# Russoul/cuda-mat

Hardware: AMD Instinct MI355X
Metric: BiCGSTAB iters/sec + SpMV effective HBM GB/s, 10M-row CSR at 1/2/4/8 GPUs (higher is better)
Workload: dtype f64

## Files before the change

### cuda_mat_amd/csrc/config.cpp

```cpp
#include "config.h"

#include <stdio.h>
#include <stdlib.h>
#include <string.h>

#include <unistd.h>

#include <mutex>
#include <set>
#include <string>

extern char **environ;

#include "common.h"

namespace cm {

namespace {

enum Kind { K_FLAG, K_INT, K_LLONG, K_ENUM, K_FAIL };

struct Option {
    const char *name;
    Kind kind;
// ... 14 lines not shown
    OPT_ENUM("SPMV_MODE", spmv_mode, "csr=0,pb=1,sell=2,pat=3", "force the CSR forms / the blocked two-phase form / SELL-C-sigma / the row-pattern dictionary"),
    OPT_FLAG("SPMV_SELL", spmv_sell, "0: keep SELL-C-sigma out of the candidates"),
    OPT_ENUM("SPMV_FORM", spmv_form, "lanes=1,tiles=2", "inside the CSR forms: lanes per row / nnz-balanced tiles"),
    OPT_INT("SPMV_LANES", spmv_lanes, 2, 64, "lanes per row, a power of two (and no stream tiles)"),
    OPT_FLAG("SPMV_COMPRESS", spmv_compress, "0: stream kernel on the plain 32-bit indices"),
    OPT_FLAG("SPMV_ALIGN", spmv_align, "0: compressed stream kernel without line-aligned copies of its value / offset streams"),
    OPT_ENUM("SPMV_TUNE", spmv_tune_full, "full=1", "time every SpMV candidate even when the column span already decides"),
    OPT_FLAG("VALUE_DICT", value_dict, "0: keep fp64 values even when the matrix has <= 256 distinct ones"),
    OPT_INT("PB_MIN_WAVES", pb_min_waves, 256, 1 << 20, "blocked form: fewest phase-2 waves"),
    OPT_INT("PB_DEPTH", pb_depth, 4, 16, "blocked form: segment loads in flight per phase-2 wave (4, 8 or 16)"),
    OPT_FLAG("POOL", pool, "0: device memory straight from hipMalloc / hipFree instead of the library's recycling pool (read once per process)"),
    OPT_FLAG("SKIP_ORIG_COPY", skip_orig_copy, "0: cudamat_solve with ILU(0) builds the blocked copy in the original index space even when its loop will run in the level-major spaces"),
    OPT_FLAG("EARLY_ANALYSIS", early_analysis, "0: cudamat_solve analyses the ILU(0) levels after the upload of the values instead of beside it"),
    OPT_INT("PB_FILL_OCC", pb_fill_occ, 0, 64, "resident waves per CU of the two-pass fill's first pass (0: 8; probing)"),
    OPT_FLAG("PB_FILL2", pb_fill2, "0: fill the blocked copy with the single-pass scatter kernel (rounds 1-4) instead of the two-pass partition"),
    OPT_INT("PB_PLACE", pb_place, 0, 2, "blocked copy of a large matrix: 1 (default): a resident solver's product stream is placed in a memory class of its own, values and indices in another (timed probe of the device's memory classes, 10-35 ms per copy: spmv_pb.hip); 2: the drop-in calls place theirs as well; 0: arrays wherever the allocator puts them"),
    OPT_INT("PB_PLACE_MAX_MS", pb_place_max_ms, 0, 60000, "PB_PLACE: what the search for an arrangement may take before the arrays are allocated as ever (ms; the slabs it allocates included -- 0.3 ms per 16 GB on most boxes, 2 s on some)"),
    OPT_FLAG("PB_PROBE_FAIL", pb_probe_fail, "1 (tests): treat the run-time LDS-order probe as failed, i.e. select the architected-order phase 2"),
    OPT_FLAG("PB_STRICT", pb_strict, "1: phase 2 adds a row's products of one wave instruction rank by rank (architected order, +10 %)"),
    {"FUSED", K_LLONG, nullptr, &Config::fused, 0, 1LL << 40, nullptr,
     "0: never fold the vector updates into the SpMVs (three launches per iteration); N: do it for every supported plan up to N rows"},
    OPT_FLAG("RESIDENT", resident, "0: never run the whole loop of a very small system in one launch"),
    OPT_INT("RESIDENT_SPIN_LIMIT", resident_spin_limit, 0, 1 << 30, "polls a grid-barrier wait of the single-launch loop may take"),
    OPT_FLAG("GUARD", guard, "1: every solve on the context runs as if CUDAMAT_FLAG_GUARD were set: restart from the true residual when rho has lost its last bit, converged = 1 only for a verified iterate (reference loops, one GPU)"),
    {"GUARD_RHO_ULPS", K_LLONG, nullptr, &Config::guard_rho_ulps, 1, 1LL << 52, nullptr,
     "guarded solves restart when |rho| <= N * 2^-52 * sum |rw_i r_i| (default 4; 2^52 fires at every iteration >= 1: tests)"},
    OPT_INT("PIPE_RR", pipe_rr, 0, 1 << 20, "residual replacement period of the pipelined loop (0: never)"),
    OPT_FLAG("TRSV_SYNCFREE", trsv_syncfree, "0: one launch per level; 1: dependency-driven launches also for narrow levels"),
    OPT_FLAG("TRSV_LDS", trsv_lds, "0: no single-workgroup LDS-resident triangular solve for small systems"),
    OPT_FLAG("TRSV_HYBRID", trsv_hybrid, "0 | 1: never / always split big factors into far (blocked SpMV) and near (dependency-driven) parts"),
// ... 151 lines not shown
```

### cuda_mat_amd/csrc/config.h

```cpp
#pragma once

namespace cm {

struct Config {
    int verbose = 0;
    int roctx = 0;
    int spmv_mode = -1;
    int spmv_sell = 1;
    int spmv_form = 0;
    int spmv_lanes = 0;
    int spmv_compress = 1;
    int spmv_align = 1;
    int spmv_tune_full = 0;
    int value_dict = 1;
    int pb_min_waves = 0;
    int pb_depth = 0;
    int pool = 1;
    int skip_orig_copy = 1;
    int early_analysis = 1;
    int pb_fill_occ = 0;
    int pb_fill2 = 1;
    int pb_place = 1;
    int pb_place_max_ms = 300;
    int pb_probe_fail = 0;
    int pb_strict = 0;
    long long fused = -1;
    int resident = 1;
    int resident_spin_limit = -1;
    int guard = 0;
    long long guard_rho_ulps = 4;
    int pipe_rr = -1;
    int trsv_syncfree = -1;
    int trsv_lds = 1;
    int trsv_hybrid = -1;
    int trsv_groups = 0;
    int trsv_lanes = 0;
// ... 26 lines not shown
```

### cuda_mat_amd/csrc/spmv_pb.h

```cpp
#pragma once
#include "kernels.h"
#include "valdict.h"

namespace cm {

constexpr int kPbMaxChunks = 16;

struct PbCols {
    int64_t per = 0;
    int chunks = 1;
    int rank = 0;
};

struct PbPlan {
    int n = 0;
    int64_t n_cols = 0;
    int64_t nnz = 0;
    int CB = 0, NCB = 0;
    int64_t per = 0;
    int chunks = 1;
    int64_t chunk_len = 0;
    int bpc = 0;
    int RB = 0, NRB = 0;
    int NW = 0;
    int SR = 0;
    int LPS = 64;
    int depth = 4;
    int NSUB = 0;
    double *pv = nullptr;
    unsigned char *pvi = nullptr;
    const double *dict = nullptr;
    int ndict = 0;
    unsigned short *pc = nullptr;
    unsigned short *pr = nullptr;
    double *P = nullptr;
    int *cstart = nullptr;
    int *col0 = nullptr;
    int *sstart = nullptr;
    int *slen = nullptr;
    int *order = nullptr;
    int part_off[kPbMaxChunks + 2] = {0};
    int placed = -1;
    int place_slabs = 0;
    double place_seconds = 0.0;
    float place_check_ms = 0.f, place_fast_ms = 0.f, place_slow_ms = 0.f;
    char place_classes[192] = {0};
    bool pc_zeroed = false;
    double build_seconds = 0.0;
};

struct PbCut {
    int per, chunks, chunk_len, bpc, CB;
};
struct PbBuild {
    PbPlan p;
    int *bins = nullptr;
    PbCut cut{};
    size_t cap = 0;
    double t0 = 0.0;
    bool verbose = false;
    bool two_pass = false;
    int place = 0;
    bool report_classes = false;
    double place_max_seconds = 0.3;
    int fill_occ = 0;
    int GB = 1, NG = 1;
    unsigned long long *smeta = nullptr;
    int *gstart = nullptr;
};
int pb_build_begin(hipStream_t st, const Config &cfg, int n, int64_t n_cols, int64_t nnz, const int *rp, const int *ci,
                   const PbCols *cols, PbBuild *b);
int pb_build_alloc(hipStream_t st, const Config &cfg, int n, int64_t n_cols, int64_t nnz, const PbCols *cols, PbBuild *b);
int pb_build_count(hipStream_t st, const Config &cfg, const int *rp, const int *ci, PbBuild *b);
// ... 17 lines not shown
```

### cuda_mat_amd/csrc/spmv_pb.hip

```cpp
#include <algorithm>
#include <map>
#include <mutex>
#include <string>
#include <vector>

#include "device.h"
#include "spmv_pb.h"

namespace cm {

typedef unsigned short u16;
constexpr int kPbBuildWaves = 4;
constexpr int kP1Threads = 1024;
constexpr int kP1Unroll = 8;
constexpr int kTileMax = 13312;
constexpr int kPbAlign = 64;

void pb_free(PbPlan *p)
{
    void *ptrs[] = {p->pv, p->pvi, p->pc, p->pr, p->P, p->cstart, p->col0, p->sstart, p->slen, p->order};
    for (void *q : ptrs)
        if (q) CM_DROP(hipFree(q));
    *p = PbPlan();
}

bool pb_candidate(hipStream_t st, int n, int64_t n_cols, int64_t nnz, const int *rp, const int *ci)
{
    (void)st; (void)rp; (void)ci;
    if (n < 65536 || nnz < (1 << 20) || n_cols * 8 < (1 << 20)) return false;
    if ((double)nnz / n < 4.0) return false;
    if ((int64_t)n > (int64_t)kMaxParts * kTileMax) return false;
    return true;
}

__device__ __forceinline__ int col_to_cb(const PbCut &c, int col)
// ... 17 lines not shown
__device__ __forceinline__ int wave_match_rank(unsigned long long *tab, int key, bool active, int lane, int nkeys, int *count_of_key_lane)
{
    if (lane < nkeys) tab[lane] = 0ULL;
    __builtin_amdgcn_fence(__ATOMIC_RELEASE, "wavefront");
    __builtin_amdgcn_wave_barrier();
    if (active) atomicOr(&tab[key], 1ULL << lane);
    __builtin_amdgcn_fence(__ATOMIC_RELEASE, "wavefront");
    __builtin_amdgcn_wave_barrier();
    const unsigned long long mine = active ? tab[key] : 0ULL;
    *count_of_key_lane = lane < nkeys ? __popcll(tab[lane]) : 0;
    __builtin_amdgcn_fence(__ATOMIC_RELEASE, "wavefront");
    __builtin_amdgcn_wave_barrier();
    return __popcll(mine & ((1ULL << lane) - 1ULL));
}

template <bool FILL>
__global__ __launch_bounds__(64 * kPbBuildWaves) void k_pb_rows(int n, const int *rp, const int *ci,
                                                               const double *val, PbCut cut, const int *col0, int NCB,
                                                               int SR, int NSUB, int *bins, double *pv, u16 *pc, u16 *pr,
                                                               const unsigned char *vidx, unsigned char *pvi, int sub0, int sub1)
{
    extern __shared__ int lds_i[];
    const int wave = threadIdx.x >> 6, lane = threadIdx.x & 63;
    const int sub = sub0 + blockIdx.x * kPbBuildWaves + wave;
    if (sub >= sub1) return;
    int *cur = lds_i + (size_t)wave * NCB;
    for (int c = lane; c < NCB; c += 64) cur[c] = FILL ? bins[(size_t)c * NSUB + sub] : 0;
    __builtin_amdgcn_fence(__ATOMIC_RELEASE, "wavefront");
    __builtin_amdgcn_wave_barrier();
    const long long row0 = (long long)sub * SR;
    const int row1 = (int)(row0 + SR < n ? row0 + SR : n);
    for (int row = (int)row0; row < row1; row++) {
        const int rs = rp[row], re = rp[row + 1];
        for (int k0 = rs; k0 < re; k0 += 64) {
            const int k = k0 + lane;
// ... 6 lines not shown
#pragma unroll
            for (int o = 1; o < 64; o <<= 1) {
                const int t = __shfl_up(hs, o, 64);
                if (lane >= o) hs = t > hs ? t : hs;
            }
            const int next = __shfl_down(cb, 1, 64);
            const bool tail = lane == 63 || next != cb;
            if (active) {
                const int base = cur[cb];
                const int rank = lane - hs;
                if (FILL) {
                    const int dest = base + rank;
                    if (pvi) pvi[dest] = vidx[k];
                    else pv[dest] = val[k];
                    pc[dest] = (u16)(col - col0[cb]);
                    pr[dest] = (u16)(row - (int)row0);
                }
                if (tail) cur[cb] = base + rank + 1;
            }
            __builtin_amdgcn_fence(__ATOMIC_RELEASE, "wavefront");
            __builtin_amdgcn_wave_barrier();
        }
    }
    if (!FILL)
        for (int c = lane; c < NCB; c += 64) bins[(size_t)c * NSUB + sub] = cur[c];
}

constexpr int kPbGroups = 32;
static_assert(kPbGroups <= 64, "one lane per group");
constexpr int kPbRpMax = 2047;
constexpr int kPbBucketMax = 2048;
// ... 98 lines not shown
        run += added;
        if (active) {
            if (sval8) sval8[dest] = vi;
            else sval[dest] = v;
            smeta[dest] = pb_pack(cb, col - (one_piece ? cb * cut.CB : col0[cb]), r);
        }
        const unsigned long long am = __ballot(active);
        rbase = __builtin_amdgcn_readlane(r, 63 - __builtin_clzll(am));
    }
}

constexpr int kPbScatterWaves = 4;
__global__ __launch_bounds__(64 * kPbScatterWaves) void k_pb_scatter(int NCB, int NSUB, const int *slen, const int *bins, int GB, int NG,
                                                                    const int *gstart, const double *sval, const unsigned char *sval8,
                                                                    const unsigned long long *smeta, double *pv, unsigned char *pvi,
                                                                    u16 *pc, u16 *pr, int sub0, int sub1)
{
    __shared__ unsigned raw_all[kPbScatterWaves][kPbBucketMax];
    __shared__ unsigned char cbl_all[kPbScatterWaves][kPbBucketMax];
    __shared__ u16 inv_all[kPbScatterWaves][kPbBucketMax];
    __shared__ unsigned long long tab_all[kPbScatterWaves][64];
    const int wave = threadIdx.x >> 6, lane = threadIdx.x & 63;
    const long long bucket = (long long)blockIdx.x * kPbScatterWaves + wave;
    const int sub = sub0 + (int)(bucket / NG), g = (int)(bucket % NG);
    if (sub >= sub1) return;
    u16 *inv = inv_all[wave];
    unsigned *raw = raw_all[wave];
    unsigned char *cbs = cbl_all[wave];
    const int start = gstart[(size_t)sub * (NG + 1) + g], len = gstart[(size_t)sub * (NG + 1) + g + 1] - start;
    if (len <= 0) return;
    const int cbid = g * GB + lane;
    const bool owner = lane < GB && cbid < NCB;
    const int cnt = owner ? slen[(size_t)sub * NCB + cbid] : 0;
    int inc = cnt;
#pragma unroll
    for (int o = 1; o < 64; o <<= 1) {
        const int t = __shfl_up(inc, o, 64);
        if (lane >= o) inc += t;
    }
    const int lbase = inc - cnt;
    const int gdst = owner ? bins[(size_t)cbid * NSUB + sub] : 0;
    const bool staged = len <= kPbBucketMax;
    int run = staged ? lbase : gdst;
    unsigned long long m_next = lane < len ? smeta[start + lane] : 0ULL;
    for (int k0 = 0; k0 < len; k0 += 64) {
        const int k = k0 + lane;
        const bool active = k < len;
        const unsigned long long m = m_next;
        m_next = k + 64 < len ? smeta[start + k + 64] : 0ULL;
        const int cbl = active ? (int)(m >> 32) - g * GB : 0;
        int added;
        const int rank = wave_match_rank(tab_all[wave], cbl, active, lane, GB, &added);
        const int r = __shfl(run, cbl, 64) + rank;
        run += added;
        if (active) {
            if (staged) { inv[r] = (u16)k; raw[k] = (unsigned)(m & 0xffffffffULL); cbs[k] = (unsigned char)cbl; }
            else {
                if (pvi) pvi[r] = sval8[start + k];
                else pv[r] = sval[start + k];
                pc[r] = (u16)((m >> 16) & 0xffff);
                pr[r] = (u16)(m & 0xffff);
            }
        }
    }
    if (!staged) return;
    __builtin_amdgcn_fence(__ATOMIC_RELEASE, "wavefront");
    __builtin_amdgcn_wave_barrier();
    for (int t0 = 0; t0 < len; t0 += 256) {
        unsigned m[4];
        double v[4];
        unsigned char vi[4];
        int dest[4];
#pragma unroll
        for (int u = 0; u < 4; u++) {
            const int t = t0 + 64 * u + lane;
            const bool active = t < len;
            const int loc = active ? (int)inv[t] : 0;
            m[u] = raw[loc];
            v[u] = 0.0;
            vi[u] = 0;
            if (active) { if (pvi) vi[u] = sval8[start + loc]; else v[u] = sval[start + loc]; }
            const int cbl = active ? (int)cbs[loc] : 0;
            dest[u] = __shfl(gdst, cbl, 64) + (t - __shfl(lbase, cbl, 64));
        }
#pragma unroll
        for (int u = 0; u < 4; u++) {
            if (t0 + 64 * u + lane < len) {
                if (pvi) pvi[dest[u]] = vi[u];
                else pv[dest[u]] = v[u];
                pc[dest[u]] = (u16)((m[u] >> 16) & 0xffff);
                pr[dest[u]] = (u16)(m[u] & 0xffff);
            }
        }
    }
}

__global__ __launch_bounds__(kBlock) void k_pb_colsum(int NSUB, const int *bins, int *colsum)
{
    __shared__ int red[kBlock / 64];
    const int *b = bins + (size_t)blockIdx.x * NSUB;
    int acc = 0;
    for (int i = threadIdx.x; i < NSUB; i += kBlock) acc += b[i];
#pragma unroll
    for (int o = 32; o > 0; o >>= 1) acc += __shfl_xor(acc, o, 64);
    if ((threadIdx.x & 63) == 0) red[threadIdx.x >> 6] = acc;
    __syncthreads();
// ... 29 lines not shown
    for (int s0 = 0; s0 < NSUB; s0 += kBlock) {
        const int sidx = s0 + threadIdx.x;
        const int cnt = sidx < NSUB ? b[sidx] : 0;
        int total;
        const int ex = block_scan_int(cnt, lds_waves, &total);
        if (sidx < NSUB) {
            const int start = run + ex;
            b[sidx] = start;
            sstart[(size_t)sidx * NCB + c] = start;
            slen[(size_t)sidx * NCB + c] = cnt;
        }
        run += total;
    }
}

static int round_blocks(int64_t n, int tile_max)
{
    int64_t m = (n + (int64_t)256 * tile_max - 1) / ((int64_t)256 * tile_max);
    if (m < 1) m = 1;
    return (int)(256 * m);
}

static void pb_scratch_free(PbBuild *b)
{
    if (b->smeta) CM_DROP(hipFree(b->smeta));
    if (b->gstart) CM_DROP(hipFree(b->gstart));
    b->smeta = nullptr;
    b->gstart = nullptr;
}

void pb_build_abort(PbBuild *b)
{
    pb_scratch_free(b);
    if (b->bins) CM_DROP(hipFree(b->bins));
    b->bins = nullptr;
    pb_free(&b->p);
}

int pb_build_begin(hipStream_t st, const Config &cfg, int n, int64_t n_cols, int64_t nnz, const int *rp, const int *ci,
                   const PbCols *cols, PbBuild *b)
{
    CM_TRY(pb_build_alloc(st, cfg, n, n_cols, nnz, cols, b));
    return pb_build_count(st, cfg, rp, ci, b);
// ... 53 lines not shown
    if (cfg.pb_depth) p.depth = cfg.pb_depth;
    if (p.NRB > kMaxParts || p.CB > 65536 || p.SR > 65536 || (size_t)p.RB * 8 > 150 * 1024 ||
        sizeof(int) * (size_t)kPbBuildWaves * p.NCB > 150 * 1024) {
        set_error("pb_build: matrix shape outside the blocked kernel's limits");
        return CUDAMAT_ERR_ARG;
    }
    const size_t nbins = (size_t)p.NCB * p.NSUB;
    int *&bins = b->bins;
    bins = nullptr;
    int rc = CUDAMAT_OK;
    do {
        if ((rc = dev_alloc(&bins, nbins))) break;
        constexpr int align = kPbAlign;
        const size_t cap = (size_t)nnz + (size_t)(align - 1) * (size_t)p.NCB + 16;
        b->cap = cap;
        if ((rc = dev_alloc(&p.cstart, (size_t)p.NCB + 1))) break;
        if ((rc = dev_alloc(&p.col0, (size_t)p.NCB + 1))) break;
        if ((rc = dev_alloc(&p.order, (size_t)p.NCB))) break;
        {
            std::vector<int> h0((size_t)p.NCB + 1), ord;
            const int per_slice = p.chunks * p.bpc;
            for (int cb = 0; cb <= p.NCB; cb++) {
                const int64_t q = cb / per_slice, ch = (cb % per_slice) / p.bpc, k = cb % p.bpc;
                int64_t in_piece = k * (int64_t)p.CB;
                if (in_piece > p.chunk_len) in_piece = p.chunk_len;
                int64_t in_slice = ch * p.chunk_len + in_piece;
                if (in_slice > p.per) in_slice = p.per;
                int64_t c0 = q * p.per + in_slice;
                if (c0 > n_cols) c0 = n_cols;
                h0[(size_t)cb] = (int)c0;
// ... 10 lines not shown
                            for (int k = 0; k < p.bpc; k++) ord.push_back((q * p.chunks + ch) * p.bpc + k);
                    p.part_off[ch + 2] = (int)ord.size();
                }
            } else {
                for (int cb = 0; cb < p.NCB; cb++) ord.push_back(cb);
                p.part_off[0] = 0;
                for (int ch = 0; ch <= p.chunks; ch++) p.part_off[ch + 1] = p.NCB;
            }
            if (hipMemcpyAsync(p.col0, h0.data(), sizeof(int) * h0.size(), hipMemcpyHostToDevice, st) != hipSuccess ||
                hipMemcpyAsync(p.order, ord.data(), sizeof(int) * ord.size(), hipMemcpyHostToDevice, st) != hipSuccess ||
                hipStreamSynchronize(st) != hipSuccess) { rc = CUDAMAT_ERR_HIP; set_error("pb column cut upload failed"); break; }
        }
        b->cut = PbCut{(int)p.per, p.chunks, (int)p.chunk_len, p.bpc, p.CB};
        if ((rc = dev_alloc(&p.sstart, nbins))) break;
        if ((rc = dev_alloc(&p.slen, nbins))) break;
        if ((rc = set_max_lds((const void *)k_pb_count))) break;
        if ((rc = set_max_lds((const void *)k_pb_rows<true>))) break;
        b->GB = 1;
        while (b->GB * kPbGroups < p.NCB) b->GB *= 2;
        b->NG = (p.NCB + b->GB - 1) / b->GB;
        b->fill_occ = cfg.pb_fill_occ;
        b->place = cfg.pb_place;
        b->place_max_seconds = 1e-3 * cfg.pb_place_max_ms;
        b->verbose = cfg.verbose != 0;
        b->report_classes = cfg.verbose >= 2;
        b->two_pass = cfg.pb_fill2 != 0 && nnz > 0 && nnz < 0x7fffffffLL && p.SR <= 65536 && b->GB <= 64;
        if (b->two_pass) {
            if (dev_alloc(&b->smeta, (size_t)nnz) != CUDAMAT_OK || dev_alloc(&b->gstart, (size_t)p.NSUB * (size_t)(b->NG + 1)) != CUDAMAT_OK) {
                if (b->smeta) CM_DROP(hipFree(b->smeta));
                b->smeta = nullptr;
// ... 10 lines not shown
    PbPlan &p = b->p;
    const int n = p.n;
    const int64_t nnz = p.nnz;
    int *bins = b->bins;
    constexpr int align = kPbAlign;
    int rc = CUDAMAT_OK;
    do {
        const PbCut cut = b->cut;
        const unsigned grid = (unsigned)((p.NSUB + kPbBuildWaves - 1) / kPbBuildWaves);
        const size_t lds = sizeof(int) * (size_t)kPbBuildWaves * p.NCB;
        hipLaunchKernelGGL(k_pb_count, dim3(grid), dim3(64 * kPbBuildWaves), lds, st, n, rp, ci, cut, p.NCB, p.SR, p.NSUB, bins, 0, p.NSUB);
        if (hipGetLastError() != hipSuccess) { rc = CUDAMAT_ERR_HIP; set_error("pb count launch failed"); break; }
        hipLaunchKernelGGL(k_pb_colsum, dim3(p.NCB), dim3(kBlock), 0, st, p.NSUB, bins, p.cstart);
        hipLaunchKernelGGL(k_pb_colscan, dim3(1), dim3(kBlock), 0, st, p.NCB, p.cstart, p.cstart, align);
        hipLaunchKernelGGL(k_pb_segscan, dim3(p.NCB), dim3(kBlock), 0, st, p.NCB, p.NSUB, p.cstart, bins, p.sstart, p.slen);
        int counted = -1;
        if (hipGetLastError() != hipSuccess ||
            hipMemcpyAsync(&counted, p.cstart + p.NCB, sizeof(int), hipMemcpyDeviceToHost, st) != hipSuccess ||
            hipStreamSynchronize(st) != hipSuccess) { rc = CUDAMAT_ERR_HIP; set_error("pb scan failed"); break; }
        if ((int64_t)counted < nnz || (int64_t)counted > nnz + (int64_t)(align - 1) * p.NCB) {
            rc = CUDAMAT_ERR_ARG; set_error("pb_build: counted %d entries, expected %lld", counted, (long long)nnz); break;
        }
        b->verbose = cfg.verbose != 0;
        b->report_classes = cfg.verbose >= 2;
    } while (0);
    if (rc) pb_build_abort(b);
    return rc;
}

__global__ __launch_bounds__(1024) void k_place_probe(const double2 *rd, double2 *wr, long n2)
{
    const long per = (n2 + gridDim.x - 1) / gridDim.x;
    const long lo = blockIdx.x * per, hi = lo + per < n2 ? lo + per : n2;
    for (long i = lo + threadIdx.x; i < hi; i += 1024) {
// ... 254 lines not shown

int pb_build_values(hipStream_t st, PbBuild *b, const ValDict *vd)
{
    PbPlan &p = b->p;
    const size_t cap = b->cap;
    const bool dict = vd && vd->n > 0;
    int rc = CUDAMAT_OK;
    if (dict && p.pv) {
        CM_DROP(hipFree(p.pv));
        p.pv = nullptr;
    }
    do {
        if (!p.P && b->place > 0 && sizeof(double) * cap >= kPlaceMinBytes) {
            void *v = nullptr, *c = nullptr, *r = nullptr, *pp = nullptr;
            bool placed = false;
            if ((rc = place_copy(st, b->verbose, b->place_max_seconds, dict ? cap : sizeof(double) * cap, sizeof(u16) * cap, sizeof(double) * cap, &v, &c, &r, &pp, &placed, &p))) break;
            if (placed) {
                if (dict) p.pvi = (unsigned char *)v; else p.pv = (double *)v;
                p.pc = (u16 *)c;
                p.pr = (u16 *)r;
                p.P = (double *)pp;
            }
        }
        if (dict) {
            if (!p.pvi && (rc = dev_alloc(&p.pvi, cap))) break;
            if (hipMemsetAsync(p.pvi, 0, cap, st) != hipSuccess) { rc = CUDAMAT_ERR_HIP; break; }
            p.dict = vd->dict;
            p.ndict = vd->n;
        } else {
            if (!p.pv && (rc = dev_alloc(&p.pv, cap))) break;
            if (hipMemsetAsync(p.pv, 0, sizeof(double) * cap, st) != hipSuccess) { rc = CUDAMAT_ERR_HIP; break; }
        }
        if (p.P && p.pc && p.pr && p.pc_zeroed) break;
        if (!p.pc && (rc = dev_alloc(&p.pc, cap))) break;
        if (!p.pr && (rc = dev_alloc(&p.pr, cap))) break;
        if (!p.P && (rc = dev_alloc(&p.P, cap))) break;
        if (kPbAlign > 1 && hipMemsetAsync(p.pc, 0, sizeof(u16) * cap, st) != hipSuccess) { rc = CUDAMAT_ERR_HIP; break; }
        p.pc_zeroed = true;
    } while (0);
    if (rc) pb_build_abort(b);
    return rc;
}

int pb_build_fill(hipStream_t st, PbBuild *b, const int *rp, const int *ci, const double *val, const ValDict *vd, int sub0, int sub1)
{
    PbPlan &p = b->p;
    if (sub1 > p.NSUB) sub1 = p.NSUB;
    if (sub1 <= sub0) return CUDAMAT_OK;
    const unsigned grid = (unsigned)((sub1 - sub0 + kPbBuildWaves - 1) / kPbBuildWaves);
    const unsigned char *vidx = p.pvi ? vd->idx : (const unsigned char *)nullptr;
    const int cfg_fill_occ = b->fill_occ;
    if (b->two_pass) {
        size_t pad = 0;
        if (cfg_fill_occ > 0) {
            const size_t per_wg = (size_t)(160 * 1024) / (size_t)((cfg_fill_occ + kPbBuildWaves - 1) / kPbBuildWaves);
            pad = per_wg > 40 * 1024 ? per_wg - 40 * 1024 : 0;
            if (pad > 64 * 1024) pad = 64 * 1024;
        }
        hipLaunchKernelGGL(k_pb_group, dim3(grid), dim3(64 * kPbBuildWaves), pad, st, p.n, rp, ci, val, vidx, b->cut, p.col0, p.NCB, p.SR,
                           p.slen, b->GB, b->NG, b->gstart, p.P, p.pvi ? (unsigned char *)p.P : (unsigned char *)nullptr, b->smeta, sub0, sub1);
        const long long buckets = (long long)(sub1 - sub0) * b->NG;
        hipLaunchKernelGGL(k_pb_scatter, dim3((unsigned)((buckets + kPbScatterWaves - 1) / kPbScatterWaves)), dim3(64 * kPbScatterWaves), 0, st,
                           p.NCB, p.NSUB, p.slen, b->bins, b->GB, b->NG, b->gstart, p.P, p.pvi ? (const unsigned char *)p.P : (const unsigned char *)nullptr,
                           b->smeta, p.pv, p.pvi, p.pc, p.pr, sub0, sub1);
    } else {
        const size_t lds = sizeof(int) * (size_t)kPbBuildWaves * p.NCB;
        hipLaunchKernelGGL(k_pb_rows<true>, dim3(grid), dim3(64 * kPbBuildWaves), lds, st, p.n, rp, ci, val, b->cut, p.col0,
                           p.NCB, p.SR, p.NSUB, b->bins, p.pv, p.pc, p.pr, vidx, p.pvi, sub0, sub1);
    }
    if (hipGetLastError() != hipSuccess) { set_error("pb fill launch failed"); pb_build_abort(b); return CUDAMAT_ERR_HIP; }
    return CUDAMAT_OK;
}

static void pb_print_plan(const PbPlan &p)
{
    const size_t nbins = (size_t)p.NCB * p.NSUB;
    std::vector<int> hl(nbins);
    if (hipMemcpy(hl.data(), p.slen, sizeof(int) * nbins, hipMemcpyDeviceToHost) != hipSuccess) return;
    long long hist[7] = {0, 0, 0, 0, 0, 0, 0}, in_long = 0;
    for (int v : hl) {
        hist[v == 0 ? 0 : v <= 8 ? 1 : v <= 24 ? 2 : v <= 48 ? 3 : v <= 64 ? 4 : v <= 128 ? 5 : 6]++;
        if (v > 64) in_long += v;
    }
    fprintf(stderr, "[cudamat] pb arrays: pv %p pvi %p pc %p pr %p P %p sstart %p slen %p cstart %p\n", (void *)p.pv, (void *)p.pvi, (void *)p.pc,
            (void *)p.pr, (void *)p.P, (void *)p.sstart, (void *)p.slen, (void *)p.cstart);
    fprintf(stderr, "[cudamat] pb plan: %d x %lld, nnz %lld, NCB %d (CB %d), NSUB %d (NW %d, SR %d), LPS %d, depth %d; segments: "
                    "empty %lld, 1-8 %lld, 9-24 %lld, 25-48 %lld, 49-64 %lld, 65-128 %lld, >128 %lld; %.1f %% of the entries in "
                    "segments longer than a wave\n",
            p.n, (long long)p.n_cols, (long long)p.nnz, p.NCB, p.CB, p.NSUB, p.NW, p.SR, p.LPS, p.depth, hist[0], hist[1], hist[2], hist[3],
            hist[4], hist[5], hist[6], 100.0 * (double)in_long / (double)(p.nnz > 0 ? p.nnz : 1));
}

static void place_report_classes(hipStream_t st, const PbPlan &p, size_t cap)
{
    if (!pool_enabled()) return;
    PlaceTimer tm(st);
    if (!tm.ok) return;
    int dev = 0;
    if (hipGetDevice(&dev) != hipSuccess) return;
    std::lock_guard<std::mutex> lock(g_place_mu);
    PlaceMemo &m = g_place[dev];
    if (m.gen != pool_generation()) { m.gen = pool_generation(); m.reset(); }
    std::vector<char *> slabs;
    std::vector<char *> scratch(3, nullptr);
    for (int k = 0; k < 4 && !(scratch[0] && scratch[1] && scratch[2]); k++) {
        char *base = nullptr;
        if (hipMalloc(&base, kPlaceSlab) != hipSuccess) { CM_DROP(hipGetLastError()); break; }
        slabs.push_back(base);
        char *seg = nullptr;
        size_t bytes = 0;
        if (!pool_segment_of(base, &seg, &bytes)) break;
        char *b0 = seg + ((size_t)(base - seg) + kPlaceBlock - 1) / kPlaceBlock * kPlaceBlock;
        for (char *q = b0; q + kPlaceBlock <= base + bytes; q += kPlaceBlock) {
            const int c = place_class_of(tm, m, q);
            if (c >= 0 && c < 3 && !scratch[c]) scratch[c] = q;
        }
    }
    struct Arr { const char *name; const char *ptr; size_t bytes; };
    const Arr arrs[4] = {{"values", p.pv ? (const char *)p.pv : (const char *)p.pvi, p.pv ? sizeof(double) * cap : cap},
                         {"col idx", (const char *)p.pc, sizeof(u16) * cap}, {"row idx", (const char *)p.pr, sizeof(u16) * cap}, {"products", (const char *)p.P, sizeof(double) * cap}};
    for (const Arr &a : arrs) {
        std::string line;
        for (size_t off = 0; off + kPlaceSample <= a.bytes; off += kPlaceSample) {
            int cls = -1;
            float worst = 0.f;
            for (int k = 0; k < 3; k++) {
                if (!scratch[k]) continue;
                const float t = tm.ms(a.ptr + off, scratch[k] + kPlaceBlock - kPlaceSample, kPlaceSample);
                if (t > worst) { worst = t; cls = k; }
            }
            line += cls < 0 || !(m.t_hi >= kPlaceGap * m.t_lo) || worst <= sqrtf(m.t_lo * m.t_hi) ? '?' : (char)('0' + cls);
        }
        fprintf(stderr, "[cudamat] pb classes: %-8s at %p, per %zu MB: %s\n", a.name, (const void *)a.ptr, kPlaceSample >> 20, line.c_str());
    }
    for (char *q : slabs) CM_DROP(hipFree(q));
}

int pb_build_end(hipStream_t st, PbBuild *b, PbPlan *out)
{
    if (hipStreamSynchronize(st) != hipSuccess) { set_error("pb fill failed"); pb_build_abort(b); return CUDAMAT_ERR_HIP; }
    if (b->verbose) pb_print_plan(b->p);
    if (b->report_classes && sizeof(double) * b->cap >= kPlaceMinBytes) place_report_classes(st, b->p, b->cap);
    pb_scratch_free(b);
    CM_DROP(hipFree(b->bins));
    b->bins = nullptr;
    b->p.build_seconds = now_s() - b->t0;
    *out = b->p;
    b->p = PbPlan();
    return CUDAMAT_OK;
}

int pb_build(hipStream_t st, const Config &cfg, int n, int64_t n_cols, int64_t nnz, const int *rp, const int *ci,
             const double *val, PbPlan *out, const PbCols *cols, const ValDict *vd)
{
    PbBuild b;
    CM_TRY(pb_build_begin(st, cfg, n, n_cols, nnz, rp, ci, cols, &b));
    CM_TRY(pb_build_values(st, &b, vd));
// ... 110 lines not shown
            double2 o;
            o.x = dv[iw & 0xffu] * xs[cw & 0xffffu];
            o.y = dv[iw >> 8] * xs[cw >> 16];
            *(double2 *)(P + kr) = o;
        } else if (kr < e) {
            P[kr] = dv[pvi[kr]] * xs[pc[kr]];
        }
    }
}

struct Pb2Args {
    int n, NCB, SR;
    const int *sstart, *slen;
    const double *P;
    const u16 *pr;
    const double *d, *xd;
    double alpha, beta;
    double *y;
    int dot;
    const double *w;
    double *parts;
    const LoopState *st;
    int strict;
    const int *xd_idx;
};

__device__ __forceinline__ void pb_seg_add(double *my, int r, double p, bool on, int lane, int group_first, bool strict)
{
    if (!strict) {
        if (on) unsafeAtomicAdd(&my[r], p);
// ... 62 lines not shown
        hipLaunchKernelGGL(k_lds_order_probe, dim3(1), dim3(64), 0, ctx->stream, flag);
        CM_HIP(hipGetLastError());
        CM_HIP(hipMemcpyAsync(&h, flag, sizeof(int), hipMemcpyDeviceToHost, ctx->stream));
        CM_HIP(hipStreamSynchronize(ctx->stream));
        if (ctx->cfg.pb_probe_fail) h = 1;
        ctx->lds_lane_order = h ? 0 : 1;
        if (h || ctx->cfg.verbose)
            fprintf(stderr, "[cudamat] LDS order probe: equal addresses of one ds_add_f64 are %s -> blocked SpMV phase 2 in its %s form\n",
                    h ? (ctx->cfg.pb_probe_fail ? "reported NOT in lane order (PB_PROBE_FAIL)" : "NOT served in lane order")
                      : "served in lane order", h ? "architected-order (PB_STRICT)" : "default");
    }
    *strict = ctx->lds_lane_order ? 0 : 1;
    return CUDAMAT_OK;
}

template <int NW, int LPS, int DEPTH, bool IDX = false>
__global__ __launch_bounds__(64 * NW) void k_pb_phase2(Pb2Args a)
{
    extern __shared__ __attribute__((aligned(16))) double yt[];
    if (a.st && a.st->state != 0) return;
    const int wave = threadIdx.x >> 6, lane = threadIdx.x & 63;
    const int sub = blockIdx.x * NW + wave;
    double *my = yt + (size_t)wave * a.SR;
    for (int i = lane; i < a.SR; i += 64) my[i] = 0.0;
    __builtin_amdgcn_fence(__ATOMIC_RELEASE, "wavefront");
    __builtin_amdgcn_wave_barrier();
    const int *ss = a.sstart + (size_t)sub * a.NCB;
    const int *sl = a.slen + (size_t)sub * a.NCB;
    for (int cb0 = 0; cb0 < a.NCB; cb0 += 64) {
        const int c = cb0 + lane;
        const int mys = c < a.NCB ? ss[c] : 0;
        const int myl = c < a.NCB ? sl[c] : 0;
        const int lim = a.NCB - cb0 < 64 ? a.NCB - cb0 : 64;
        const bool grouped = LPS < 64 && !__any(myl > LPS);
        if (!grouped) {
            for (int j = 0; j < lim; j += DEPTH) {
                int s[DEPTH], l[DEPTH];
                double pv4[DEPTH];
                int r4[DEPTH];
#pragma unroll
                for (int u = 0; u < DEPTH; u++) {
                    s[u] = __builtin_amdgcn_readlane(mys, (j + u) & 63);
                    l[u] = __builtin_amdgcn_readlane(myl, (j + u) & 63);
                }
#pragma unroll
                for (int u = 0; u < DEPTH; u++) {
                    const bool on = lane < l[u];
                    pv4[u] = on ? a.P[s[u] + lane] : 0.0;
                    r4[u] = on ? (int)a.pr[s[u] + lane] : 0;
                }
#pragma unroll
                for (int u = 0; u < DEPTH; u++) {
                    pb_seg_add(my, r4[u], pv4[u], lane < l[u], lane, 0, a.strict != 0);
                    for (int off0 = 64; off0 < l[u]; off0 += 64) {
                        const int off = off0 + lane;
                        const bool on = off < l[u];
                        pb_seg_add(my, on ? (int)a.pr[s[u] + off] : 0, on ? a.P[s[u] + off] : 0.0, on, lane, 0, a.strict != 0);
                    }
                }
            }
        } else {
            constexpr int G = 64 / LPS;
            const int g = lane / LPS, li = lane % LPS;
            for (int j = 0; j < lim; j += DEPTH * G) {
                int s[DEPTH], l[DEPTH];
                double pv4[DEPTH];
                int r4[DEPTH];
#pragma unroll
                for (int u = 0; u < DEPTH; u++) {
                    const int cbi = j + u * G + g;
                    s[u] = __shfl(mys, cbi & 63, 64);
                    l[u] = cbi < 64 ? __shfl(myl, cbi & 63, 64) : 0;
                }
#pragma unroll
                for (int u = 0; u < DEPTH; u++) {
                    const bool on = li < l[u];
                    pv4[u] = on ? a.P[s[u] + li] : 0.0;
                    r4[u] = on ? (int)a.pr[s[u] + li] : 0;
                }
#pragma unroll
                for (int u = 0; u < DEPTH; u++) {
                    if (!a.strict) {
                        if (li < l[u]) unsafeAtomicAdd(&my[r4[u]], pv4[u]);
                    } else {
#pragma unroll
                        for (int gg = 0; gg < G; gg++)
                            pb_seg_add(my, r4[u], pv4[u], g == gg && li < l[u], lane, gg * LPS, true);
                    }
                }
            }
        }
    }
    __builtin_amdgcn_fence(__ATOMIC_RELEASE, "wavefront");
    __builtin_amdgcn_wave_barrier();
    double acc0 = 0.0, acc1 = 0.0;
    const long long row0 = (long long)sub * a.SR;
    for (int i = lane; i < a.SR && row0 + i < a.n; i += 64) {
#pragma clang fp contract(off)
        const int row = (int)(row0 + i);
        double sum = my[i];
        if (a.d) {
            const double dx = a.d[row] * a.xd[IDX ? a.xd_idx[row] : row];
            sum = sum + dx;
        }
        double out = a.alpha * sum;
// ... 62 lines not shown
    return launch_pb_phase1_blocks(st, p, a, p.order, p.part_off[part], p.part_off[part + 1]);
}

int launch_spmv_pb(hipStream_t st, const PbPlan &p, const SpmvArgs &a)
{
    CM_TRY(launch_pb_check(st, a));
    CM_TRY(launch_pb_phase1(st, p, a, -1));
    return launch_pb_phase2(st, p, a);
}

int launch_pb_phase2(hipStream_t st, const PbPlan &p, const SpmvArgs &a)
{
    Pb2Args b;
    b.n = p.n; b.NCB = p.NCB; b.SR = p.SR;
    b.sstart = p.sstart; b.slen = p.slen;
    b.P = p.P; b.pr = p.pr;
    b.d = a.d; b.xd = a.xd; b.xd_idx = a.xd_idx;
    b.alpha = a.alpha; b.beta = a.beta;
    b.y = a.y; b.dot = a.dot; b.w = a.w; b.parts = a.parts;
    b.st = a.loop.st;
    b.strict = a.pb_strict;
    const size_t lds = sizeof(double) * ((size_t)p.NW * p.SR + 2 * (size_t)p.NW);
    const bool idx = b.d && b.xd_idx;
#define CM_P2D(NWV, LPSV, DV, IDXV)                                                                               \
    do {                                                                                                          \
        CM_TRY(set_max_lds((const void *)k_pb_phase2<NWV, LPSV, DV, IDXV>));                                     \
        hipLaunchKernelGGL((k_pb_phase2<NWV, LPSV, DV, IDXV>), dim3(p.NRB), dim3(64 * NWV), lds, st, b);         \
    } while (0)
#define CM_P2(NWV, LPSV)                                                                                  \
    do {                                                                                                  \
        if (idx && p.depth >= 16) CM_P2D(NWV, LPSV, 16, true);                                            \
        else if (idx) CM_P2D(NWV, LPSV, 4, true);                                                         \
        else if (p.depth >= 16) CM_P2D(NWV, LPSV, 16, false);                                             \
        else if (p.depth >= 8) CM_P2D(NWV, LPSV, 8, false);                                               \
        else CM_P2D(NWV, LPSV, 4, false);                                                                 \
    } while (0)
#define CM_P2_LPS(NWV)                                           \
    do {                                                         \
        if (p.LPS == 16) CM_P2(NWV, 16);                         \
        else if (p.LPS == 32) CM_P2(NWV, 32);                    \
        else CM_P2(NWV, 64);                                     \
    } while (0)
    switch (p.NW) {
    case 4:  CM_P2_LPS(4); break;
    case 8:  CM_P2_LPS(8); break;
    default: CM_P2_LPS(16); break;
    }
#undef CM_P2_LPS
#undef CM_P2
#undef CM_P2D
    CM_HIP(hipGetLastError());
    return CUDAMAT_OK;
}

}
```

Baseline: 182.3.

## Store blocked-copy row indices as one contiguous aligned run per phase-2 wave

The blocked SpMV copy now stores its 16-bit row indices in a separate layout: one 128-byte-aligned run per phase-2 wave (sub-block), read front to back. Before, they sat in the entries' (column block, sub-block) order. Build kernels scatter each row index through a per-(sub, column-block) offset table. Phase 2 walks a running cursor instead of the segment start, so each wave reads its row indices sequentially for better locality. The cost is extra build-time scans, a slightly larger row-index array, and a depth-8 phase-2 variant that now falls back to depth 4 when this layout is on.

```diff
diff --git a/cuda_mat_amd/csrc/config.cpp b/cuda_mat_amd/csrc/config.cpp
--- a/cuda_mat_amd/csrc/config.cpp
+++ b/cuda_mat_amd/csrc/config.cpp
@@ -52,6 +52,7 @@
     OPT_FLAG("EARLY_ANALYSIS", early_analysis, "0: cudamat_solve analyses the ILU(0) levels after the upload of the values instead of beside it"),
     OPT_INT("PB_FILL_OCC", pb_fill_occ, 0, 64, "resident waves per CU of the two-pass fill's first pass (0: 8; probing)"),
     OPT_FLAG("PB_FILL2", pb_fill2, "0: fill the blocked copy with the single-pass scatter kernel (rounds 1-4) instead of the two-pass partition"),
+    OPT_FLAG("PB_WAVE_ROWS", pb_wave_rows, "0: the blocked copy keeps its row indices in the order of its entries (column block, sub-block) instead of one 128-byte-aligned run per phase-2 wave, read front to back (read when the copy is built)"),
     OPT_INT("PB_PLACE", pb_place, 0, 2, "blocked copy of a large matrix: 1 (default): a resident solver's product stream is placed in a memory class of its own, values and indices in another (timed probe of the device's memory classes, 10-35 ms per copy: spmv_pb.hip); 2: the drop-in calls place theirs as well; 0: arrays wherever the allocator puts them"),
     OPT_INT("PB_PLACE_MAX_MS", pb_place_max_ms, 0, 60000, "PB_PLACE: what the search for an arrangement may take before the arrays are allocated as ever (ms; the slabs it allocates included -- 0.3 ms per 16 GB on most boxes, 2 s on some)"),
     OPT_FLAG("PB_PROBE_FAIL", pb_probe_fail, "1 (tests): treat the run-time LDS-order probe as failed, i.e. select the architected-order phase 2"),
diff --git a/cuda_mat_amd/csrc/config.h b/cuda_mat_amd/csrc/config.h
--- a/cuda_mat_amd/csrc/config.h
+++ b/cuda_mat_amd/csrc/config.h
@@ -20,6 +20,7 @@
     int early_analysis = 1;
     int pb_fill_occ = 0;
     int pb_fill2 = 1;
+    int pb_wave_rows = 1;
     int pb_place = 1;
     int pb_place_max_ms = 300;
     int pb_probe_fail = 0;
diff --git a/cuda_mat_amd/csrc/spmv_pb.h b/cuda_mat_amd/csrc/spmv_pb.h
--- a/cuda_mat_amd/csrc/spmv_pb.h
+++ b/cuda_mat_amd/csrc/spmv_pb.h
@@ -38,6 +38,8 @@
     int *col0 = nullptr;
     int *sstart = nullptr;
     int *slen = nullptr;
+    int wave_rows = 0;
+    int *wbase = nullptr;
     int *order = nullptr;
     int part_off[kPbMaxChunks + 2] = {0};
     int placed = -1;
@@ -57,6 +59,8 @@
     int *bins = nullptr;
     PbCut cut{};
     size_t cap = 0;
+    size_t cap_rows = 0;
+    int *wdelta = nullptr;
     double t0 = 0.0;
     bool verbose = false;
     bool two_pass = false;
diff --git a/cuda_mat_amd/csrc/spmv_pb.hip b/cuda_mat_amd/csrc/spmv_pb.hip
--- a/cuda_mat_amd/csrc/spmv_pb.hip
+++ b/cuda_mat_amd/csrc/spmv_pb.hip
@@ -18,7 +18,7 @@
 
 void pb_free(PbPlan *p)
 {
-    void *ptrs[] = {p->pv, p->pvi, p->pc, p->pr, p->P, p->cstart, p->col0, p->sstart, p->slen, p->order};
+    void *ptrs[] = {p->pv, p->pvi, p->pc, p->pr, p->P, p->cstart, p->col0, p->sstart, p->slen, p->wbase, p->order};
     for (void *q : ptrs)
         if (q) CM_DROP(hipFree(q));
     *p = PbPlan();
@@ -66,11 +66,24 @@
     return __popcll(mine & ((1ULL << lane) - 1ULL));
 }
 
+__device__ __forceinline__ int wave_scan_excl(int v, int lane, int *total)
+{
+    int inc = v;
+#pragma unroll
+    for (int o = 1; o < 64; o <<= 1) {
+        const int t = __shfl_up(inc, o, 64);
+        if (lane >= o) inc += t;
+    }
+    *total = __builtin_amdgcn_readlane(inc, 63);
+    return inc - v;
+}
+
 template <bool FILL>
 __global__ __launch_bounds__(64 * kPbBuildWaves) void k_pb_rows(int n, const int *rp, const int *ci,
                                                                const double *val, PbCut cut, const int *col0, int NCB,
                                                                int SR, int NSUB, int *bins, double *pv, u16 *pc, u16 *pr,
-                                                               const unsigned char *vidx, unsigned char *pvi, int sub0, int sub1)
+                                                               const unsigned char *vidx, unsigned char *pvi, const int *wdelta,
+                                                               int sub0, int sub1)
 {
     extern __shared__ int lds_i[];
     const int wave = threadIdx.x >> 6, lane = threadIdx.x & 63;
@@ -107,7 +120,7 @@
                     if (pvi) pvi[dest] = vidx[k];
                     else pv[dest] = val[k];
                     pc[dest] = (u16)(col - col0[cb]);
-                    pr[dest] = (u16)(row - (int)row0);
+                    pr[dest + (wdelta ? wdelta[(size_t)sub * NCB + cb] : 0)] = (u16)(row - (int)row0);
                 }
                 if (tail) cur[cb] = base + rank + 1;
             }
@@ -236,7 +249,7 @@
 __global__ __launch_bounds__(64 * kPbScatterWaves) void k_pb_scatter(int NCB, int NSUB, const int *slen, const int *bins, int GB, int NG,
                                                                     const int *gstart, const double *sval, const unsigned char *sval8,
                                                                     const unsigned long long *smeta, double *pv, unsigned char *pvi,
-                                                                    u16 *pc, u16 *pr, int sub0, int sub1)
+                                                                    u16 *pc, u16 *pr, const int *wdelta, int sub0, int sub1)
 {
     __shared__ unsigned raw_all[kPbScatterWaves][kPbBucketMax];
     __shared__ unsigned char cbl_all[kPbScatterWaves][kPbBucketMax];
@@ -262,6 +275,7 @@
     }
     const int lbase = inc - cnt;
     const int gdst = owner ? bins[(size_t)cbid * NSUB + sub] : 0;
+    const int wd = owner && wdelta ? wdelta[(size_t)sub * NCB + cbid] : 0;
     const bool staged = len <= kPbBucketMax;
     int run = staged ? lbase : gdst;
     unsigned long long m_next = lane < len ? smeta[start + lane] : 0ULL;
@@ -274,6 +288,7 @@
         int added;
         const int rank = wave_match_rank(tab_all[wave], cbl, active, lane, GB, &added);
         const int r = __shfl(run, cbl, 64) + rank;
+        const int rw = r + __shfl(wd, cbl, 64);
         run += added;
         if (active) {
             if (staged) { inv[r] = (u16)k; raw[k] = (unsigned)(m & 0xffffffffULL); cbs[k] = (unsigned char)cbl; }
@@ -281,7 +296,7 @@
                 if (pvi) pvi[r] = sval8[start + k];
                 else pv[r] = sval[start + k];
                 pc[r] = (u16)((m >> 16) & 0xffff);
-                pr[r] = (u16)(m & 0xffff);
+                pr[rw] = (u16)(m & 0xffff);
             }
         }
     }
@@ -292,7 +307,7 @@
         unsigned m[4];
         double v[4];
         unsigned char vi[4];
-        int dest[4];
+        int dest[4], destr[4];
 #pragma unroll
         for (int u = 0; u < 4; u++) {
             const int t = t0 + 64 * u + lane;
@@ -304,6 +319,7 @@
             if (active) { if (pvi) vi[u] = sval8[start + loc]; else v[u] = sval[start + loc]; }
             const int cbl = active ? (int)cbs[loc] : 0;
             dest[u] = __shfl(gdst, cbl, 64) + (t - __shfl(lbase, cbl, 64));
+            destr[u] = dest[u] + __shfl(wd, cbl, 64);
         }
 #pragma unroll
         for (int u = 0; u < 4; u++) {
@@ -311,7 +327,7 @@
                 if (pvi) pvi[dest[u]] = vi[u];
                 else pv[dest[u]] = v[u];
                 pc[dest[u]] = (u16)((m[u] >> 16) & 0xffff);
-                pr[dest[u]] = (u16)(m[u] & 0xffff);
+                pr[destr[u]] = (u16)(m[u] & 0xffff);
             }
         }
     }
@@ -371,6 +387,23 @@
     }
 }
 
+__global__ __launch_bounds__(64 * kPbBuildWaves) void k_pb_wdelta(int NCB, int NSUB, const int *sstart, const int *slen, const int *wbase,
+                                                                 int *wdelta)
+{
+    const int wave = threadIdx.x >> 6, lane = threadIdx.x & 63;
+    const int sub = blockIdx.x * kPbBuildWaves + wave;
+    if (sub >= NSUB) return;
+    int run = wbase[sub];
+    for (int c0 = 0; c0 < NCB; c0 += 64) {
+        const int c = c0 + lane;
+        const int cnt = c < NCB ? slen[(size_t)sub * NCB + c] : 0;
+        int total;
+        const int ex = wave_scan_excl(cnt, lane, &total);
+        if (c < NCB) wdelta[(size_t)sub * NCB + c] = run + ex - sstart[(size_t)sub * NCB + c];
+        run += total;
+    }
+}
+
 static int round_blocks(int64_t n, int tile_max)
 {
     int64_t m = (n + (int64_t)256 * tile_max - 1) / ((int64_t)256 * tile_max);
@@ -382,8 +415,10 @@
 {
     if (b->smeta) CM_DROP(hipFree(b->smeta));
     if (b->gstart) CM_DROP(hipFree(b->gstart));
+    if (b->wdelta) CM_DROP(hipFree(b->wdelta));
     b->smeta = nullptr;
     b->gstart = nullptr;
+    b->wdelta = nullptr;
 }
 
 void pb_build_abort(PbBuild *b)
@@ -467,6 +502,9 @@
         constexpr int align = kPbAlign;
         const size_t cap = (size_t)nnz + (size_t)(align - 1) * (size_t)p.NCB + 16;
         b->cap = cap;
+        const size_t cap_w = (size_t)nnz + (size_t)(align - 1) * (size_t)p.NSUB + 16;
+        p.wave_rows = cfg.pb_wave_rows != 0 && nnz > 0 && cap_w < (size_t)0x7fffffff ? 1 : 0;
+        b->cap_rows = p.wave_rows && cap_w > cap ? cap_w : cap;
         if ((rc = dev_alloc(&p.cstart, (size_t)p.NCB + 1))) break;
         if ((rc = dev_alloc(&p.col0, (size_t)p.NCB + 1))) break;
         if ((rc = dev_alloc(&p.order, (size_t)p.NCB))) break;
@@ -507,6 +545,8 @@
         b->cut = PbCut{(int)p.per, p.chunks, (int)p.chunk_len, p.bpc, p.CB};
         if ((rc = dev_alloc(&p.sstart, nbins))) break;
         if ((rc = dev_alloc(&p.slen, nbins))) break;
+        if (p.wave_rows && (rc = dev_alloc(&p.wbase, (size_t)p.NSUB + 1))) break;
+        if (p.wave_rows && (rc = dev_alloc(&b->wdelta, nbins))) break;
         if ((rc = set_max_lds((const void *)k_pb_count))) break;
         if ((rc = set_max_lds((const void *)k_pb_rows<true>))) break;
         b->GB = 1;
@@ -547,10 +587,19 @@
         hipLaunchKernelGGL(k_pb_colsum, dim3(p.NCB), dim3(kBlock), 0, st, p.NSUB, bins, p.cstart);
         hipLaunchKernelGGL(k_pb_colscan, dim3(1), dim3(kBlock), 0, st, p.NCB, p.cstart, p.cstart, align);
         hipLaunchKernelGGL(k_pb_segscan, dim3(p.NCB), dim3(kBlock), 0, st, p.NCB, p.NSUB, p.cstart, bins, p.sstart, p.slen);
-        int counted = -1;
+        int counted = -1, wave_slots = 0;
+        if (p.wave_rows) {
+            hipLaunchKernelGGL(k_pb_colsum, dim3(p.NSUB), dim3(kBlock), 0, st, p.NCB, p.slen, p.wbase);
+            hipLaunchKernelGGL(k_pb_colscan, dim3(1), dim3(kBlock), 0, st, p.NSUB, p.wbase, p.wbase, align);
+            hipLaunchKernelGGL(k_pb_wdelta, dim3(grid), dim3(64 * kPbBuildWaves), 0, st, p.NCB, p.NSUB, p.sstart, p.slen, p.wbase, b->wdelta);
+            if (hipMemcpyAsync(&wave_slots, p.wbase + p.NSUB, sizeof(int), hipMemcpyDeviceToHost, st) != hipSuccess) { rc = CUDAMAT_ERR_HIP; set_error("pb scan failed"); break; }
+        }
         if (hipGetLastError() != hipSuccess ||
             hipMemcpyAsync(&counted, p.cstart + p.NCB, sizeof(int), hipMemcpyDeviceToHost, st) != hipSuccess ||
             hipStreamSynchronize(st) != hipSuccess) { rc = CUDAMAT_ERR_HIP; set_error("pb scan failed"); break; }
+        if (p.wave_rows && (wave_slots < 0 || (size_t)wave_slots > b->cap_rows)) {
+            rc = CUDAMAT_ERR_ARG; set_error("pb_build: %d row-index slots in wave order, room for %zu", wave_slots, b->cap_rows); break;
+        }
         if ((int64_t)counted < nnz || (int64_t)counted > nnz + (int64_t)(align - 1) * p.NCB) {
             rc = CUDAMAT_ERR_ARG; set_error("pb_build: counted %d entries, expected %lld", counted, (long long)nnz); break;
         }
@@ -835,7 +884,7 @@
         if (!p.P && b->place > 0 && sizeof(double) * cap >= kPlaceMinBytes) {
             void *v = nullptr, *c = nullptr, *r = nullptr, *pp = nullptr;
             bool placed = false;
-            if ((rc = place_copy(st, b->verbose, b->place_max_seconds, dict ? cap : sizeof(double) * cap, sizeof(u16) * cap, sizeof(double) * cap, &v, &c, &r, &pp, &placed, &p))) break;
+            if ((rc = place_copy(st, b->verbose, b->place_max_seconds, dict ? cap : sizeof(double) * cap, sizeof(u16) * b->cap_rows, sizeof(double) * cap, &v, &c, &r, &pp, &placed, &p))) break;
             if (placed) {
                 if (dict) p.pvi = (unsigned char *)v; else p.pv = (double *)v;
                 p.pc = (u16 *)c;
@@ -854,7 +903,7 @@
         }
         if (p.P && p.pc && p.pr && p.pc_zeroed) break;
         if (!p.pc && (rc = dev_alloc(&p.pc, cap))) break;
-        if (!p.pr && (rc = dev_alloc(&p.pr, cap))) break;
+        if (!p.pr && (rc = dev_alloc(&p.pr, b->cap_rows))) break;
         if (!p.P && (rc = dev_alloc(&p.P, cap))) break;
         if (kPbAlign > 1 && hipMemsetAsync(p.pc, 0, sizeof(u16) * cap, st) != hipSuccess) { rc = CUDAMAT_ERR_HIP; break; }
         p.pc_zeroed = true;
@@ -883,11 +932,11 @@
         const long long buckets = (long long)(sub1 - sub0) * b->NG;
         hipLaunchKernelGGL(k_pb_scatter, dim3((unsigned)((buckets + kPbScatterWaves - 1) / kPbScatterWaves)), dim3(64 * kPbScatterWaves), 0, st,
                            p.NCB, p.NSUB, p.slen, b->bins, b->GB, b->NG, b->gstart, p.P, p.pvi ? (const unsigned char *)p.P : (const unsigned char *)nullptr,
-                           b->smeta, p.pv, p.pvi, p.pc, p.pr, sub0, sub1);
+                           b->smeta, p.pv, p.pvi, p.pc, p.pr, b->wdelta, sub0, sub1);
     } else {
         const size_t lds = sizeof(int) * (size_t)kPbBuildWaves * p.NCB;
         hipLaunchKernelGGL(k_pb_rows<true>, dim3(grid), dim3(64 * kPbBuildWaves), lds, st, p.n, rp, ci, val, b->cut, p.col0,
-                           p.NCB, p.SR, p.NSUB, b->bins, p.pv, p.pc, p.pr, vidx, p.pvi, sub0, sub1);
+                           p.NCB, p.SR, p.NSUB, b->bins, p.pv, p.pc, p.pr, vidx, p.pvi, b->wdelta, sub0, sub1);
     }
     if (hipGetLastError() != hipSuccess) { set_error("pb fill launch failed"); pb_build_abort(b); return CUDAMAT_ERR_HIP; }
     return CUDAMAT_OK;
@@ -903,8 +952,9 @@
         hist[v == 0 ? 0 : v <= 8 ? 1 : v <= 24 ? 2 : v <= 48 ? 3 : v <= 64 ? 4 : v <= 128 ? 5 : 6]++;
         if (v > 64) in_long += v;
     }
-    fprintf(stderr, "[cudamat] pb arrays: pv %p pvi %p pc %p pr %p P %p sstart %p slen %p cstart %p\n", (void *)p.pv, (void *)p.pvi, (void *)p.pc,
-            (void *)p.pr, (void *)p.P, (void *)p.sstart, (void *)p.slen, (void *)p.cstart);
+    fprintf(stderr, "[cudamat] pb arrays: pv %p pvi %p pc %p pr %p P %p sstart %p slen %p cstart %p wbase %p (row indices %s)\n", (void *)p.pv,
+            (void *)p.pvi, (void *)p.pc, (void *)p.pr, (void *)p.P, (void *)p.sstart, (void *)p.slen, (void *)p.cstart, (void *)p.wbase,
+            p.wave_rows ? "one run per phase-2 wave" : "in the entries' order");
     fprintf(stderr, "[cudamat] pb plan: %d x %lld, nnz %lld, NCB %d (CB %d), NSUB %d (NW %d, SR %d), LPS %d, depth %d; segments: "
                     "empty %lld, 1-8 %lld, 9-24 %lld, 25-48 %lld, 49-64 %lld, 65-128 %lld, >128 %lld; %.1f %% of the entries in "
                     "segments longer than a wave\n",
@@ -912,7 +962,7 @@
             hist[4], hist[5], hist[6], 100.0 * (double)in_long / (double)(p.nnz > 0 ? p.nnz : 1));
 }
 
-static void place_report_classes(hipStream_t st, const PbPlan &p, size_t cap)
+static void place_report_classes(hipStream_t st, const PbPlan &p, size_t cap, size_t cap_rows)
 {
     if (!pool_enabled()) return;
     PlaceTimer tm(st);
@@ -939,7 +989,7 @@
     }
     struct Arr { const char *name; const char *ptr; size_t bytes; };
     const Arr arrs[4] = {{"values", p.pv ? (const char *)p.pv : (const char *)p.pvi, p.pv ? sizeof(double) * cap : cap},
-                         {"col idx", (const char *)p.pc, sizeof(u16) * cap}, {"row idx", (const char *)p.pr, sizeof(u16) * cap}, {"products", (const char *)p.P, sizeof(double) * cap}};
+                         {"col idx", (const char *)p.pc, sizeof(u16) * cap}, {"row idx", (const char *)p.pr, sizeof(u16) * cap_rows}, {"products", (const char *)p.P, sizeof(double) * cap}};
     for (const Arr &a : arrs) {
         std::string line;
         for (size_t off = 0; off + kPlaceSample <= a.bytes; off += kPlaceSample) {
@@ -961,7 +1011,7 @@
 {
     if (hipStreamSynchronize(st) != hipSuccess) { set_error("pb fill failed"); pb_build_abort(b); return CUDAMAT_ERR_HIP; }
     if (b->verbose) pb_print_plan(b->p);
-    if (b->report_classes && sizeof(double) * b->cap >= kPlaceMinBytes) place_report_classes(st, b->p, b->cap);
+    if (b->report_classes && sizeof(double) * b->cap >= kPlaceMinBytes) place_report_classes(st, b->p, b->cap, b->cap_rows);
     pb_scratch_free(b);
     CM_DROP(hipFree(b->bins));
     b->bins = nullptr;
@@ -1102,6 +1152,7 @@
     const int *sstart, *slen;
     const double *P;
     const u16 *pr;
+    const int *wbase;
     const double *d, *xd;
     double alpha, beta;
     double *y;
@@ -1194,7 +1245,13 @@
     return CUDAMAT_OK;
 }
 
-template <int NW, int LPS, int DEPTH, bool IDX = false>
+template <bool WR>
+__device__ __forceinline__ int pb_row_index(const Pb2Args &a, int seg_start, int row_start, int k)
+{
+    return (int)a.pr[(WR ? row_start : seg_start) + k];
+}
+
+template <int NW, int LPS, int DEPTH, bool IDX = false, bool WR = false>
 __global__ __launch_bounds__(64 * NW) void k_pb_phase2(Pb2Args a)
 {
     extern __shared__ __attribute__((aligned(16))) double yt[];
@@ -1207,6 +1264,7 @@
     __builtin_amdgcn_wave_barrier();
     const int *ss = a.sstart + (size_t)sub * a.NCB;
     const int *sl = a.slen + (size_t)sub * a.NCB;
+    int wrun = WR ? __builtin_amdgcn_readfirstlane(a.wbase[sub]) : 0;
     for (int cb0 = 0; cb0 < a.NCB; cb0 += 64) {
         const int c = cb0 + lane;
         const int mys = c < a.NCB ? ss[c] : 0;
@@ -1218,6 +1276,7 @@
                 int s[DEPTH], l[DEPTH];
                 double pv4[DEPTH];
                 int r4[DEPTH];
+                int wadd = wrun;
 #pragma unroll
                 for (int u = 0; u < DEPTH; u++) {
                     s[u] = __builtin_amdgcn_readlane(mys, (j + u) & 63);
@@ -1227,7 +1286,8 @@
                 for (int u = 0; u < DEPTH; u++) {
                     const bool on = lane < l[u];
                     pv4[u] = on ? a.P[s[u] + lane] : 0.0;
-                    r4[u] = on ? (int)a.pr[s[u] + lane] : 0;
+                    r4[u] = on ? pb_row_index<WR>(a, s[u], wrun, lane) : 0;
+                    if (WR) wrun += l[u];
                 }
 #pragma unroll
                 for (int u = 0; u < DEPTH; u++) {
@@ -1235,11 +1295,14 @@
                     for (int off0 = 64; off0 < l[u]; off0 += 64) {
                         const int off = off0 + lane;
                         const bool on = off < l[u];
-                        pb_seg_add(my, on ? (int)a.pr[s[u] + off] : 0, on ? a.P[s[u] + off] : 0.0, on, lane, 0, a.strict != 0);
+                        pb_seg_add(my, on ? pb_row_index<WR>(a, s[u], wadd, off) : 0, on ? a.P[s[u] + off] : 0.0, on, lane, 0, a.strict != 0);
                     }
+                    if (WR) wadd += l[u];
                 }
             }
         } else {
+            int myw = 0, total = 0;
+            if (WR) myw = wrun + wave_scan_excl(myl, lane, &total);
             constexpr int G = 64 / LPS;
             const int g = lane / LPS, li = lane % LPS;
             for (int j = 0; j < lim; j += DEPTH * G) {
@@ -1255,8 +1318,9 @@
 #pragma unroll
                 for (int u = 0; u < DEPTH; u++) {
                     const bool on = li < l[u];
+                    const int wu = WR ? __shfl(myw, (j + u * G + g) & 63, 64) : 0;
                     pv4[u] = on ? a.P[s[u] + li] : 0.0;
-                    r4[u] = on ? (int)a.pr[s[u] + li] : 0;
+                    r4[u] = on ? pb_row_index<WR>(a, s[u], wu, li) : 0;
                 }
 #pragma unroll
                 for (int u = 0; u < DEPTH; u++) {
@@ -1269,6 +1333,7 @@
                     }
                 }
             }
+            wrun += total;
         }
     }
     __builtin_amdgcn_fence(__ATOMIC_RELEASE, "wavefront");
@@ -1361,7 +1426,7 @@
     Pb2Args b;
     b.n = p.n; b.NCB = p.NCB; b.SR = p.SR;
     b.sstart = p.sstart; b.slen = p.slen;
-    b.P = p.P; b.pr = p.pr;
+    b.P = p.P; b.pr = p.pr; b.wbase = p.wbase;
     b.d = a.d; b.xd = a.xd; b.xd_idx = a.xd_idx;
     b.alpha = a.alpha; b.beta = a.beta;
     b.y = a.y; b.dot = a.dot; b.w = a.w; b.parts = a.parts;
@@ -1369,17 +1434,22 @@
     b.strict = a.pb_strict;
     const size_t lds = sizeof(double) * ((size_t)p.NW * p.SR + 2 * (size_t)p.NW);
     const bool idx = b.d && b.xd_idx;
+#define CM_P2W(NWV, LPSV, DV, IDXV, WRV)                                                                          \
+    do {                                                                                                          \
+        CM_TRY(set_max_lds((const void *)k_pb_phase2<NWV, LPSV, DV, IDXV, WRV>));                                \
+        hipLaunchKernelGGL((k_pb_phase2<NWV, LPSV, DV, IDXV, WRV>), dim3(p.NRB), dim3(64 * NWV), lds, st, b);    \
+    } while (0)
 #define CM_P2D(NWV, LPSV, DV, IDXV)                                                                               \
     do {                                                                                                          \
-        CM_TRY(set_max_lds((const void *)k_pb_phase2<NWV, LPSV, DV, IDXV>));                                     \
-        hipLaunchKernelGGL((k_pb_phase2<NWV, LPSV, DV, IDXV>), dim3(p.NRB), dim3(64 * NWV), lds, st, b);         \
+        if (p.wave_rows) CM_P2W(NWV, LPSV, DV, IDXV, true);                                                       \
+        else CM_P2W(NWV, LPSV, DV, IDXV, false);                                                                  \
     } while (0)
 #define CM_P2(NWV, LPSV)                                                                                  \
     do {                                                                                                  \
         if (idx && p.depth >= 16) CM_P2D(NWV, LPSV, 16, true);                                            \
         else if (idx) CM_P2D(NWV, LPSV, 4, true);                                                         \
         else if (p.depth >= 16) CM_P2D(NWV, LPSV, 16, false);                                             \
-        else if (p.depth >= 8) CM_P2D(NWV, LPSV, 8, false);                                               \
+        else if (p.depth >= 8 && !p.wave_rows) CM_P2W(NWV, LPSV, 8, false, false);                        \
         else CM_P2D(NWV, LPSV, 4, false);                                                                 \
     } while (0)
 #define CM_P2_LPS(NWV)                                           \
@@ -1396,6 +1466,7 @@
 #undef CM_P2_LPS
 #undef CM_P2
 #undef CM_P2D
+#undef CM_P2W
     CM_HIP(hipGetLastError());
     return CUDAMAT_OK;
 }
```

Measured after the change: 182.9, median of 6. Within noise of the previous version (+0.3%).
